# jeremy-collins/sd-video-gen

Hardware: AMD Instinct MI355X
Metric: generated frames/sec at 50 DDIM denoise steps, 512x512 (higher is better)
Workload: dtype fp16; 1 GPU; configs[2]: 1_16_kitti_L1_64 F=64, 64x64 latents -> 512x512 VAE passes, 50-step DDIM; --denoise --denoise_start_step 0, guidance_scale 0; SD-v1.4 UNet at 64x64 latents, VAE enc/dec at 512x512; clips_per_gpu=56, streams_per_gpu=2, pred_frames=1, global_clips=56, parallelism=clip-sharded dp1, weights=seeded random init (SD v1.4 architecture, 1_16_kitti_L1_64)

## Files before the change

### include/svg_hip.h

```cpp
#ifndef SVG_HIP_H
#define SVG_HIP_H

#include <stdint.h>

#ifdef __cplusplus
extern "C" {
#endif

typedef struct svg_ctx svg_ctx;

enum svg_model { SVG_TRANSFORMER = 0, SVG_VAE = 1, SVG_UNET = 2, SVG_CLIP_TEXT = 3, SVG_MINILM = 4, SVG_I3D = 5 };
enum svg_status { SVG_OK = 0, SVG_ERR_RUNTIME = -1, SVG_ERR_INVALID = -2 };

int svg_create(int device_id, svg_ctx** out);
void svg_destroy(svg_ctx* ctx);
const char* svg_last_error(svg_ctx* ctx);
const char* svg_version(void);
void svg_env_refresh(void);

int svg_model_configure(svg_ctx* ctx, int model, const char* kv);
int svg_load_weight(svg_ctx* ctx, int model, const char* name, const float* data,
                    const int64_t* shape, int ndim);
int svg_finalize(svg_ctx* ctx, int model, int64_t* n_params);
const char* svg_model_dtype(svg_ctx* ctx, int model);
// ... 139 lines not shown
  int64_t vt_bs;
  const uint16_t* A2;
  int lda2, k_split;
  float* gn_part;
  float* ln_part;
  int ln_tiles;
} svg_gemm_desc;
int svg_op_gemm_ex(svg_ctx* ctx, const svg_gemm_desc* desc, int* path, void* stream);
int svg_op_gemm_plan(svg_ctx* ctx, const svg_gemm_desc* desc, int* plan);
int svg_op_ff_fused(svg_ctx* ctx, const uint16_t* x, const float* ln_gamma, const float* ln_beta, const float* w1,
                    const float* b1, const float* w2, const float* b2, const uint16_t* residual, uint16_t* out, int M,
                    int C, void* stream);
int svg_op_xattn_fused(svg_ctx* ctx, const uint16_t* x, const uint16_t* a, const uint16_t* r, const float* wp, const float* bp,
                       const float* ln_gamma, const float* ln_beta, const float* wq, const uint16_t* k, const uint16_t* vt, int Lp,
                       const float* wo, const float* bo, uint16_t* out, int M, int rows_per_sample, int L, void* stream);
int svg_op_dropout_mask(svg_ctx* ctx, uint64_t seed, int site, float p, float* out, int64_t n, void* stream);
int svg_op_xf_gemm_tn(svg_ctx* ctx, const float* dY, int ldy, const float* X, int ldx, float* dW, float* db, int M, int N, int K,
                      int accumulate, void* stream);
int svg_op_xf_gemm_nn(svg_ctx* ctx, const float* dY, int ldy, const float* W, float* out, int M, int N, int K, const float* gate,
                      float gate_scale, const float* add, int* splits, void* stream);
int svg_op_xf_relu_drop(svg_ctx* ctx, const float* h, float* r, int64_t n, uint64_t seed, int site, float p, void* stream);
int svg_op_xf_add_ln_train(svg_ctx* ctx, const float* x, const float* r, uint64_t seed, int site, float p, const float* gamma,
                           const float* beta, float* y, float* xhat, float* rstd, int M, int d, float eps, void* stream);
int svg_op_xf_ln_bwd(svg_ctx* ctx, const float* dy, const float* xhat, const float* rstd, const float* gamma, float* dz, float* dz_drop,
                     uint64_t seed, int site, float p, float* dgamma, float* dbeta, int M, int d, int accumulate, void* stream);
int svg_op_xf_attention_train(svg_ctx* ctx, const float* q, int ldq, const float* k, const float* v, int ldk, const float* mask, float* o,
                              float* P, int Tq, int Tk, int B, int heads, int hd, uint64_t seed, int site, float p, void* stream);
int svg_op_xf_attention_bwd(svg_ctx* ctx, const float* dout, const float* q, int ldq, const float* k, const float* v, int ldk,
                            const float* P, float* dq, int lddq, float* dk, float* dv, int lddk, int Tq, int Tk, int B, int heads, int hd,
                            uint64_t seed, int site, float p, void* stream);
// ... 104 lines not shown
int svg_op_conv3x3_gn_f16(svg_ctx* ctx, const uint16_t* x, const float* w_oihw, const float* bias, const float* gamma,
                          const float* beta, uint16_t* conv_out, uint16_t* gn_out, int B, int H, int W, int Cin, int Cout,
                          int groups, float eps, int silu, int* used_epilogue_stats, void* stream);
int svg_op_gemm_lnstats_f16(svg_ctx* ctx, const uint16_t* A, const uint16_t* W, const float* bias, const uint16_t* residual,
                            uint16_t* C, int M, int N, int K, int batch, float* rs, float* rm, int* used, void* stream);
int svg_op_gemm_ex_f16(svg_ctx* ctx, const svg_gemm_desc* desc, int* path, void* stream);
int svg_op_gemm_plan_f16(svg_ctx* ctx, const svg_gemm_desc* desc, int* plan);
int svg_op_gemm_cat_f16(svg_ctx* ctx, const uint16_t* A, const uint16_t* A2, const uint16_t* W, const float* bias, uint16_t* C,
                        int M, int N, int K, int k_split, void* stream);
int svg_op_ff_fused_f16(svg_ctx* ctx, const uint16_t* x, const float* ln_gamma, const float* ln_beta, const float* w1,
                        const float* b1, const float* w2, const float* b2, const uint16_t* residual, uint16_t* out, int M, int C,
                        void* stream);
int svg_op_xattn_fused_f16(svg_ctx* ctx, const uint16_t* x, const uint16_t* a, const uint16_t* r, const float* wp, const float* bp,
                           const float* ln_gamma, const float* ln_beta, const float* wq, const uint16_t* k, const uint16_t* vt, int Lp,
                           const float* wo, const float* bo, uint16_t* out, int M, int rows_per_sample, int L, void* stream);
int svg_op_conv3x3_mx_f16(svg_ctx* ctx, const uint16_t* x, const float* w_oihw, const float* bias, const uint16_t* residual,
                          uint16_t* out, uint8_t* q_out, uint8_t* s_out, int B, int H, int W, int Cin, int Cout, int mode, void* stream);
int svg_op_quant_mx_f16(svg_ctx* ctx, const uint16_t* x, uint8_t* q, uint8_t* scales, int64_t rows, int K, void* stream);
int svg_op_gemm_fp8_f16(svg_ctx* ctx, const uint16_t* A, const uint16_t* W, const float* bias, const uint16_t* residual, void* C,
                        int M, int N, int K, int act, int out_f32, void* stream);
int svg_op_quant_act_mx_f16(svg_ctx* ctx, const uint16_t* x, uint8_t* q, uint8_t* scales, int64_t P, int C, void* stream);
int svg_op_conv3x3_mx_ex_f16(svg_ctx* ctx, const svg_conv_mx_desc* desc, int* path, void* stream);
int svg_op_gemm_fp8_ex_f16(svg_ctx* ctx, const uint16_t* A, const uint16_t* W, const float* bias, const uint16_t* residual, void* C,
                           int M, int N, int K, int act, int out_f32, int ldc, int ldr, int* path, void* stream);
int svg_op_groupnorm_f16(svg_ctx* ctx, const uint16_t* x, const float* gamma, const float* beta, uint16_t* out, int B, int HW,
                         int C, int groups, float eps, int silu, void* stream);
int svg_op_conv3x3_f32s_f16(svg_ctx* ctx, const uint16_t* x, const float* w_oihw, const float* bias, const uint16_t* residual,
                            const float* residual_f32, float* out, const float* gamma, const float* beta, uint16_t* gn_out, int B, int H,
                            int W, int Cin, int Cout, int mode, int groups, float eps, int silu, int* halo_width, int* used_epilogue_stats,
                            void* stream);
// ... 83 lines not shown
```

### sd-video-gen_amd/_lib.py

```python
import ctypes as C
import os

import torch

_HERE = os.path.dirname(os.path.abspath(__file__))
LIB_PATH = os.environ.get("SVG_LIB") or os.path.join(_HERE, "libsvg_hip.so")

SVG_TRANSFORMER, SVG_VAE, SVG_UNET, SVG_CLIP_TEXT, SVG_MINILM, SVG_I3D = 0, 1, 2, 3, 4, 5
SVG_ERR_RUNTIME, SVG_ERR_INVALID = -1, -2
SAMPLERS = {"ddim": 0, "dpmpp_2m": 1, "lms": 2}


def sampler_id(name):
    if name not in SAMPLERS:
        raise ValueError("unknown sampler %r (one of %s)" % (name, ", ".join(SAMPLERS)))
    return SAMPLERS[name]

_lib = None

_vp, _i, _f, _i64 = C.c_void_p, C.c_int, C.c_float, C.c_int64

SVG_TENSOR_PARAM, SVG_TENSOR_GRAD, SVG_TENSOR_EXP_AVG, SVG_TENSOR_EXP_AVG_SQ, SVG_TENSOR_EMA = 0, 1, 2, 3, 4
SVG_BACKWARD_ACCUMULATE = 2

# ... 93 lines not shown
    "svg_sample_loop": [_vp, _i, _vp, _i, _i, _i, _vp, _i, _i, _i, _f, _vp, _vp, _vp],
    "svg_dpmpp_step": [_vp, _vp, _vp, _vp, _vp, _vp, _i64, _i, _i, _i, _vp],
    "svg_lms_coefs": [_i, _i, _vp, _vp, _vp, _vp, _vp],
    "svg_lms_step": [_vp, _vp, _vp, _vp, _vp, _i64, _i, _i, _vp],
    "svg_resize_bilinear_f32": [_vp, _vp, _i, _i, _i, _vp, _i, _i, _vp],
    "svg_resize_nearest_u8": [_vp, _vp, _i, _i, _i, _i, _vp, _i, _i, _vp],
    "svg_op_gemm": [_vp, _vp, _vp, _vp, _vp, _vp, _i, _i, _i, _i, _i, _vp],
    "svg_op_conv3x3": [_vp, _vp, _vp, _vp, _vp, _i, _i, _i, _i, _i, _i, _vp],
    "svg_op_conv3x3_gn": [_vp, _vp, _vp, _vp, _vp, _vp, _vp, _vp, _i, _i, _i, _i, _i, _i, _f, _i, C.POINTER(_i), _vp],
    "svg_op_gemm_lnstats": [_vp, _vp, _vp, _vp, _vp, _vp, _i, _i, _i, _i, _vp, _vp, C.POINTER(_i), _vp],
    "svg_op_gemm_cat": [_vp, _vp, _vp, _vp, _vp, _vp, _i, _i, _i, _i, _vp],
    "svg_op_gemm_ex": [_vp, C.POINTER(GemmDesc), C.POINTER(_i), _vp],
    "svg_op_gemm_plan": [_vp, C.POINTER(GemmDesc), C.POINTER(_i)],
    "svg_op_ff_fused": [_vp, _vp, _vp, _vp, _vp, _vp, _vp, _vp, _vp, _vp, _i, _i, _vp],
    "svg_op_xattn_fused": [_vp, _vp, _vp, _vp, _vp, _vp, _vp, _vp, _vp, _vp, _vp, _i, _vp, _vp, _vp, _i, _i, _i, _vp],
    "svg_op_dropout_mask": [_vp, C.c_uint64, _i, _f, _vp, _i64, _vp],
    "svg_op_xf_gemm_tn": [_vp, _vp, _i, _vp, _i, _vp, _vp, _i, _i, _i, _i, _vp],
    "svg_op_xf_gemm_nn": [_vp, _vp, _i, _vp, _vp, _i, _i, _i, _vp, _f, _vp, C.POINTER(_i), _vp],
    "svg_op_xf_relu_drop": [_vp, _vp, _vp, _i64, C.c_uint64, _i, _f, _vp],
    "svg_op_xf_add_ln_train": [_vp, _vp, _vp, C.c_uint64, _i, _f, _vp, _vp, _vp, _vp, _vp, _i, _i, _f, _vp],
    "svg_op_xf_ln_bwd": [_vp, _vp, _vp, _vp, _vp, _vp, _vp, C.c_uint64, _i, _f, _vp, _vp, _i, _i, _i, _vp],
    "svg_op_xf_attention_train": [_vp, _vp, _i, _vp, _vp, _i, _vp, _vp, _vp, _i, _i, _i, _i, _i, C.c_uint64, _i, _f, _vp],
    "svg_op_xf_attention_bwd": [_vp, _vp, _vp, _i, _vp, _vp, _i, _vp, _vp, _i, _vp, _vp, _i, _i, _i, _i, _i, _i, C.c_uint64, _i, _f, _vp],
    "svg_op_xf_embed_post_train": [_vp, _vp, _vp, _vp, _vp, _i, _vp, _i, _i, _i, _f, C.c_uint64, _i, _f, _vp],
    "svg_op_xf_embed_post_bwd": [_vp, _vp, _vp, _i, _i, _i, _i, _f, C.c_uint64, _i, _f, _vp],
    "svg_op_xf_criterion": [_vp, _vp, _vp, _vp, C.POINTER(_f), _i, _i, _i, _i, _i, _i, _f, _f, _f, _f, _f, _f, _vp],
    "svg_op_conv3d": [_vp, _vp, _i, _i, _i, _i, _i, _vp, _vp, _vp, _i64, _i, _i, _i, C.POINTER(_i), C.POINTER(_i), _i, C.POINTER(_i), _vp],
    "svg_op_pack_conv3d": [_vp, _vp, _vp, _vp, _vp, _vp, _vp, _vp, _vp, _i, _i, _i, _i, _f, _vp],
    "svg_op_maxpool3d_same": [_vp, _vp, _vp, _i64, _i, _i, _i, _i, _i, C.POINTER(_i), C.POINTER(_i), C.POINTER(_i), _vp],
    "svg_op_avgpool_thw": [_vp, _vp, _vp, _i, _i, _i, _i, _i, _vp],
# ... 54 lines not shown
    "svg_op_xf_embed_tokens": [_vp, _vp, _vp, _vp, _vp, _i, _i, _i, _i, _vp],
    "svg_op_xf_embed_bert": [_vp, _vp, _vp, _vp, _vp, _vp, _i, _i, _i, _i, _vp],
    "svg_op_xf_mean_pool_norm": [_vp, _vp, _vp, _vp, _i, _i, _i, _vp],
    "svg_op_xf_walk": [_vp, C.POINTER(WalkStage), _i, _i, _i, C.POINTER(_i), _vp],
    "svg_prof_enable": [_vp, _i],
    "svg_prof_reset": [_vp],
    "svg_prof_report": [_vp, C.c_char_p, _i],
    "svg_workspace_bytes": [_vp],
    "svg_transformer_status": [_vp],
    "svg_workspace_growths": [_vp],
    "svg_reserve_workspace": [_vp, _i64],
    "svg_plan_begin": [_vp],
    "svg_plan_end": [_vp, C.POINTER(_i64)],
    "svg_debug_captures_active": [],
}
for _n in ("gemm", "gemm_ex", "gemm_plan", "conv3x3", "conv3x3_gn", "conv3x3_mx", "conv3x3_mx_ex", "gemm_fp8_ex", "quant_act_mx", "gemm_lnstats", "gemm_cat", "ff_fused", "xattn_fused", "quant_mx", "gemm_fp8", "groupnorm", "layernorm",
           "attention", "attention_ex", "vae_attention", "conv3x3_f32s", "groupnorm_f32", "groupnorm_ex", "groupnorm_mx", "gn_fold_weights", "ln_stats",
           "softmax_rows", "rowsum", "img_to_act", "nchw_to_act", "actf32_pad_h16", "concat_channels", "f32_to_h16", "f32_to_h16_x8", "h16_to_f32",
           "timestep_embed"):
    SIGNATURES["svg_op_%s_f16" % _n] = SIGNATURES["svg_op_" + _n]
SIGNATURES["svg_model_dtype"] = [_vp, _i]
_RESTYPES = {"svg_destroy": None, "svg_env_refresh": None, "svg_model_dtype": C.c_char_p, "svg_last_error": C.c_char_p, "svg_version": C.c_char_p,
             "svg_workspace_bytes": _i64, "svg_workspace_growths": _i64}


def host_cpu_quota():
    n = len(os.sched_getaffinity(0)) if hasattr(os, "sched_getaffinity") else (os.cpu_count() or 1)
    limited = False
    for path in (os.environ.get("SVG_CGROUP_CPU_MAX", "/sys/fs/cgroup/cpu.max"),):
        try:
            q, p = open(path).read().split()
# ... 486 lines not shown
```

### sd-video-gen_amd/csrc/kernels.h

```cpp
#pragma once
#include "common.h"
#include "gemm_tiles.h"

namespace SDNS {

enum AMode { A_DENSE = 0, A_CONV_S1 = 1, A_CONV_S2P1 = 2, A_CONV_S2ASYM = 3, A_CONV_UP2 = 4, A_CONV_SMALLC = 5 };
enum Act { ACT_NONE = 0, ACT_SILU = 1, ACT_GELU = 2, ACT_GEGLU = 3 };

struct GemmArgs {
  const h16* A = nullptr;
  int amode = A_DENSE;
  int lda = 0;
  const h16* A2 = nullptr;
  int lda2 = 0, k_split = 0;
  int H = 0, W = 0, Cin = 0;
  int Ho = 0, Wo = 0;
  const h16* Wt = nullptr;
  int ldb = 0;
  int n_valid = 0;
  void* C = nullptr;
  int ldc = 0;
  int M = 0, N = 0, K = 0;
  int batch = 1;
  int64_t sA = 0, sB = 0, sC = 0;
// ... 59 lines not shown
void pack_conv3x3_mx(const float* w_oihw, uint8_t* q, uint8_t* sc, int O, int I, int Npad, int Cp, hipStream_t s);
struct Fp8ConvPath { int bn = 0, tn_major = 0, workgroups = 0; };
void conv_halo_fp8(svg_ctx* ctx, const uint8_t* A8, const uint8_t* As, const uint8_t* W8, const uint8_t* Ws, int Npad, const GemmArgs& g, hipStream_t s,
                   Fp8ConvPath* path = nullptr);

bool ff_fused_supported(int C, int M);
bool xattn_fused_supported(int C, int heads, int M, int rows_per_sample, int L);
int64_t xattn_kv_pack_elems(int N);
void xattn_pack_q(const float* w, const float* gamma, const float* beta, h16* Wq, float* sq, float* bq, int perm, hipStream_t s);
bool xattn_chain_enabled();
void xattn_pack_o(const float* w, h16* Wo, hipStream_t s);
void xattn_pack_kv(const h16* K, int ldk, int64_t k_bs, const h16* Vt, int ldv, int64_t v_bs, h16* Kp, h16* Vp, int N, int L, hipStream_t s);
void xattn_fused(svg_ctx* ctx, const h16* X, int ldx, const h16* R, int ldr, const h16* Wp, const float* bp, const float* rs, const float* rm,
                 const h16* Wq, const float* sq, const float* bq, const h16* Kp, const h16* Vp, const h16* Wo, const float* bo, h16* out, int ldo,
                 int M, int rows_per_sample, int L, hipStream_t s);
void pack_ff2_perm(const float* w, h16* out, int N, int K, hipStream_t s);
void ff_fused(svg_ctx* ctx, const h16* X, int ldx, const h16* W1, const float* b1, const float* s1,
              const h16* W2p, const float* b2, const h16* residual, int ldr, h16* out, int ldo, int M, hipStream_t s);
void pack_conv3x3(const float* w_oihw, h16* out, int O, int I, int Opad, int Ipad, hipStream_t s);
void pack_linear(const float* w, h16* out, int N, int K, int Npad, hipStream_t s);
void fold_ln_weights(float* w, const float* bias_in, const float* gamma, const float* beta, float* bias_out, int N, int K, hipStream_t s);
void rowsum_h16(const h16* w, float* out, int N, int K, hipStream_t s);
void ln_stats(svg_ctx* ctx, const h16* x, float* rs, float* rm, int M, int C, float eps, hipStream_t s);
void pack_geglu(const float* w, const float* b, h16* wout, float* bout, int F, int K, hipStream_t s);

void ln_finish(svg_ctx* ctx, const float* part, int tiles, float* rs, float* rm, int M, int C, float eps, hipStream_t s);
struct GnStats {
  const float* part = nullptr;
  int tiles_per_sample = 0;
  bool valid() const { return part != nullptr && tiles_per_sample > 0; }
// ... 129 lines not shown
```

### sd-video-gen_amd/csrc/models.h

```cpp
#pragma once
#include "kernels.h"
#include "sampler.h"
#include <algorithm>
#include <initializer_list>
#include <memory>

struct WeightStore {
  std::unordered_map<std::string, Weight> map;
  void put(svg_ctx* ctx, const std::string& name, const float* data, const int64_t* shape, int ndim);
  const Weight& get(const std::string& name) const;
  const Weight& get(const std::string& name, std::initializer_list<int64_t> shape) const;
  bool has(const std::string& name) const { return map.count(name) != 0; }
  void release(const std::string& name);
  void clear();
  int64_t total_params() const;
};

std::unordered_map<std::string, std::vector<int64_t>> parse_kv(const char* kv);

template <typename F>
inline void run_planned(svg_ctx* ctx, F&& body) {
  ctx->arena.reset();
  ctx->arena.dry = true;
  ctx->arena.high = 0;
// ... 175 lines not shown
  void decode(svg_ctx* ctx, const float* z, int N, int h, int w, uint8_t* img_out, int outH, int outW, float* float_out,
              hipStream_t s) override;
};

struct XfBlockW {
  NormW gn, ln1, ln2, ln3;
  PackedLinear proj_in, proj_out, qk1, v1, o1, q2, k2, v2, o2, ff1, ff2;
  PackedLinear qkv1;
  float* proj_in_f32 = nullptr;
  h16* ff2p = nullptr;
  h16* xq = nullptr; float* xq_s = nullptr; float* xq_b = nullptr;
  h16* xqp = nullptr;
  h16* xo = nullptr;
  int C = 0;
};
struct KvCache {
  struct Slot { h16* p = nullptr; int64_t cap = 0; };
  std::vector<Slot> k, vt;
  std::vector<Slot> kp, vp;
  bool valid = false;
};

struct UnetModel : UnetIface {
  KvCache kv;
  std::vector<int> block_out{320, 640, 1280, 1280};
  std::vector<int> attn{1, 1, 1, 0};
  int layers = 2, heads = 8, ctx_dim = 768, groups = 32, in_ch = 4, out_ch = 4;
  int fp8 = 0;
  const char* dtype() const override { return SD_F16 ? "fp16" : "bf16"; }
  int temb_dim = 0;
  PackedLinear time1, time2, temb_all;
  ConvW conv_in, conv_out; NormW norm_out;
  std::vector<std::vector<ResW>> down_res; std::vector<std::vector<XfBlockW>> down_attn; std::vector<ConvW> down_s;
  ResW mid0, mid1; XfBlockW mid_attn;
  std::vector<std::vector<ResW>> up_res; std::vector<std::vector<XfBlockW>> up_attn; std::vector<ConvW> up_s;
  void configure(const char* kv) override;
// ... 60 lines not shown
```

### sd-video-gen_amd/csrc/sd_ops.cpp

```cpp
#include "models.h"
#include "../../include/svg_hip.h"
#include <cstdlib>

#if SD_F16
#define SVG_OP(name) name##_f16
#else
#define SVG_OP(name) name
#endif
#define API_BEGIN try {
#define API_END(ctx)                                   \
  return 0;                                            \
  }                                                    \
  catch (const std::exception& e) { return svg_fail(ctx, e); }

using namespace SDNS;

static ConvW stage_conv(svg_ctx* ctx, const float* w_oihw, const float* bias, int Cin, int Cout, bool mx, hipStream_t s) {
  ConvW cw;
  cw.Cin = Cin; cw.Cout = Cout; cw.Opad = (int)align_up(Cout, 4);
  const int64_t nw = (int64_t)Cout * Cin * 9;
  if (!mx) cw.w = ctx->arena.get<h16>((int64_t)cw.Opad * 9 * Cin);
  float* wdev = ctx->arena.get<float>(nw);
  cw.b = ctx->arena.get<float>(cw.Opad);
  if (mx) {
// ... 311 lines not shown
      xattn_pack_q(wqd, gd, bd, Wq, sq, bq, a ? 1 : 0, s);
      xattn_pack_o(wod, Wo, s);
      xattn_pack_kv((const h16*)k, C, (int64_t)L * C, (const h16*)vt, Lp, (int64_t)C * Lp, kp, vp, N, L, s);
      if (a) {
        HIP_OK(hipMemcpyAsync(wpd, wp, (size_t)C * C * 4, hipMemcpyDefault, s));
        HIP_OK(hipMemcpyAsync(bpd, bp, (size_t)C * 4, hipMemcpyDefault, s));
        pack_linear(wpd, Wp, C, C, C, s);
      }
    }
    if (a) xattn_fused(ctx, (const h16*)a, C, (const h16*)r, C, Wp, bpd, nullptr, nullptr, Wq, sq, bq, kp, vp, Wo, bod, (h16*)out, C, M, rows_per_sample, L, s);
    else xattn_fused(ctx, (const h16*)x, C, nullptr, 0, nullptr, nullptr, nullptr, nullptr, Wq, sq, bq, kp, vp, Wo, bod, (h16*)out, C, M, rows_per_sample, L, s);
  });
  API_END(ctx)
}

int SVG_OP(svg_op_quant_mx)(svg_ctx* ctx, const uint16_t* x, uint8_t* q, uint8_t* scales, int64_t rows, int K, void* stream) {
  API_BEGIN
  quant_mx_h16(ctx, (const h16*)x, K, q, scales, rows, K, (hipStream_t)stream);
  API_END(ctx)
}

int SVG_OP(svg_op_quant_act_mx)(svg_ctx* ctx, const uint16_t* x, uint8_t* q, uint8_t* scales, int64_t P, int C, void* stream) {
  API_BEGIN
  SVG_CHECK(x && q && scales && P > 0 && C > 0 && C % 32 == 0, "quant_act_mx op: P %lld C %d unsupported (C %% 32 must be 0)", (long long)P, C);
  quant_act_mx(ctx, (const h16*)x, C, q, scales, P, (hipStream_t)stream);
  API_END(ctx)
}

int SVG_OP(svg_op_gemm_fp8)(svg_ctx* ctx, const uint16_t* A, const uint16_t* W, const float* bias, const uint16_t* residual, void* C, int M, int N,
                    int K, int act, int out_f32, void* stream) {
// ... 321 lines not shown
```

### sd-video-gen_amd/csrc/sdnet.cpp

```cpp
#include "models.h"
#include <algorithm>
#include <cstdlib>

namespace SDNS {

static int64_t chunk_limit() {
  const int64_t full = (1LL << 31) - 1;
  const int64_t v = svg_env_i64("SVG_CHUNK_LIMIT", full);
  return v > 0 && v < full ? v : full;
}

float* keep_f32(svg_ctx* ctx, WeightStore& ws, const std::string& name, int64_t numel) {
  const Weight& w = ws.get(name);
  SVG_CHECK(w.numel == numel, "weight %s has %lld elements, expected %lld", name.c_str(), (long long)w.numel, (long long)numel);
  return w.f32;
}

ConvW load_conv3x3(svg_ctx* ctx, WeightStore& ws, const std::string& prefix, int Cin, int Cout, hipStream_t s, bool fp8) {
  const Weight& w = ws.get(prefix + ".weight", {Cout, Cin, 3, 3});
  ConvW cw;
  cw.Cout = Cout;
  cw.Opad = (int)align_up(Cout, 4);
  cw.Cin = (Cin < 64) ? 8 : Cin;
  SVG_CHECK(Cin <= 8 || Cin % 64 == 0, "conv %s: Cin=%d must be <= 8 or a multiple of 64", prefix.c_str(), Cin);
// ... 211 lines not shown
void vt_proj_into(svg_ctx* ctx, const PackedLinear& wv, const h16* src, int B, int rows, int rows_pad, int K, h16* vt, hipStream_t s,
                  const float* ln_rs, const float* ln_rm) {
  const int C = wv.N;
  GemmArgs g;
  g.A = wv.w; g.lda = K; g.Wt = src; g.ldb = K; g.M = C; g.N = rows_pad; g.n_valid = rows; g.K = K;
  g.batch = B; g.sA = 0; g.sB = (int64_t)rows * K; g.sC = (int64_t)C * rows_pad;
  g.C = vt; g.ldc = rows_pad;
  SVG_CHECK((wv.ln_s != nullptr) == (ln_rs != nullptr), "vt_proj: LayerNorm-folded weights need the token statistics");
  if (wv.b) { g.bias = wv.b; g.bias_row = 1; }
  if (ln_rs) {
    g.ln_rs = ln_rs; g.ln_rm = ln_rm; g.ln_s = wv.ln_s; g.ln_swapped = 1; g.ln_zstride = rows;
  }
  gemm_auto(ctx, g, s, PK_GEMM);
}

void sd_init_device() {
  gemm_init_device();
  gemm_pp_init_device();
  gemm_ws_init_device();
  vae_attn_init_device();
  conv_halo_init_device();
  ff_fused_init_device();
  xattn_fused_init_device();
  gemm_fp8_init_device();
  conv_halo_fp8_init_device();
}

}
```

### sd-video-gen_amd/csrc/unet.cpp

```cpp
#include "models.h"
#include <algorithm>
#include <chrono>
#include <cstdlib>
#include <thread>

namespace SDNS {

void UnetModel::configure(const char* kv) {
  auto m = parse_kv(kv);
  auto geti = [&](const char* k, int& dst) { if (m.count(k)) dst = (int)m[k][0]; };
  if (m.count("block_out")) { block_out.clear(); for (auto v : m["block_out"]) block_out.push_back((int)v); }
  if (m.count("attn")) { attn.clear(); for (auto v : m["attn"]) attn.push_back((int)v); }
  geti("layers", layers); geti("heads", heads); geti("ctx_dim", ctx_dim); geti("groups", groups);
  geti("in_ch", in_ch); geti("out_ch", out_ch);
  fp8 = 0; geti("fp8", fp8);
  ready = false;
}

namespace {

struct TembCollector {
  std::vector<std::string> prefixes;
  std::vector<int> couts;
  int total = 0;
// ... 346 lines not shown
      if (!fused) {
        linear(ctx, h, C, b.qk1, qk, 2 * C, M, s, stat);
        vt = ctx->arena.get<h16>((int64_t)N * C * HWp);
        vt_proj_into(ctx, b.v1, h, N, HW, HWp, C, vt, s, rs, rm);
      }
      attn_core(qk, 2 * C, qk + C, 2 * C, (int64_t)HW * 2 * C, vt, HWp, (int64_t)C * HWp, ao, C, HW, HW);
      ctx->arena.pop();
    }
    h16* h1 = ctx->arena.get<h16>(P * C);
    const bool xa_one = b.xq && xattn_fused_supported(C, m->heads, M, HW, L);
    const bool xa_chain = xa_one && xattn_chain_enabled() && b.o1.K == C && b.o1.N == C;
    LinearOpts o1, o2;
    o1.residual = h; o1.ldr = C; o1.ln = xa_one ? nullptr : &le;
    if (!xa_chain) linear(ctx, ao, C, b.o1, h1, C, M, s, o1);
    h16* h2 = ctx->arena.get<h16>(P * C);
    if (!xa_one) row_stats(h1);
    {
      ctx->arena.push();
      h16* q = xa_one ? nullptr : ctx->arena.get<h16>(P * C);
      if (!xa_one) linear(ctx, h1, C, b.q2, q, C, M, s, stat);
      const int idx = xf_idx++;
      const int64_t kn = (int64_t)N * L * C, vn = (int64_t)N * C * Lp;
      const bool grow_cache = cache && (SVG_LAUNCHING(ctx) || ctx->plan_only);
      auto kv_buf = [&](std::vector<KvCache::Slot> KvCache::*which, int64_t n) -> h16* {
        if (!cache) return ctx->arena.get<h16>(n);
        std::vector<KvCache::Slot>& v = cache->*which;
        if (grow_cache) {
          if ((int)v.size() <= idx) v.resize(idx + 1);
          if (v[idx].cap < n) { v[idx].p = (h16*)ctx->dalloc(n * sizeof(h16)); v[idx].cap = n; cache->valid = false; }
        }
        if (idx < (int)v.size() && v[idx].p) return v[idx].p;
        return (h16*)(uintptr_t)0x1000;
      };
      h16* k = kv_buf(&KvCache::k, kn);
      h16* vt = kv_buf(&KvCache::vt, vn);
      const int64_t pn = xattn_kv_pack_elems(N);
      h16* kp = xa_one ? kv_buf(&KvCache::kp, pn) : nullptr;
      h16* vp = xa_one ? kv_buf(&KvCache::vp, pn) : nullptr;
      if (!(cache && cache->valid && SVG_LAUNCHING(ctx))) {
        linear(ctx, ctxb, m->ctx_dim, b.k2, k, C, N * L, s);
        vt_proj_into(ctx, b.v2, ctxb, N, L, Lp, m->ctx_dim, vt, s);
        if (xa_one && SVG_LAUNCHING(ctx)) xattn_pack_kv(k, C, (int64_t)L * C, vt, Lp, (int64_t)C * Lp, kp, vp, N, L, s);
      }
      if (xa_chain) xattn_fused(ctx, ao, C, h, C, b.o1.w, b.o1.b, nullptr, nullptr, b.xqp, b.xq_s, b.xq_b, kp, vp, b.xo, b.o2.b, h2, C, M, HW, L, s);
      else if (xa_one) xattn_fused(ctx, h1, C, nullptr, 0, nullptr, nullptr, nullptr, nullptr, b.xq, b.xq_s, b.xq_b, kp, vp, b.xo, b.o2.b, h2, C, M, HW, L, s);
      else attn_core(q, C, k, C, (int64_t)L * C, vt, Lp, (int64_t)C * Lp, ao, C, HW, L);
      ctx->arena.pop();
    }
    o2.residual = h1; o2.ldr = C; o2.ln = &le;
    if (!xa_one) linear(ctx, ao, C, b.o2, h2, C, M, s, o2);
    const bool ff_one = b.ff2p && ff_fused_supported(C, M);
    if (!ff_one) row_stats(h2);
    {
      if (ff_one) {
        ff_fused(ctx, h2, C, b.ff1.w, b.ff1.b, b.ff1.ln_s, b.ff2p, b.ff2.b, h2, C, h, C, M, s);
      } else {
        ctx->arena.push();
        h16* g = ctx->arena.get<h16>((int64_t)M * 4 * C);
        LinearOpts f1, f2;
        f1.act = ACT_GEGLU; f1.ln_rs = rs; f1.ln_rm = rm;
        f2.residual = h2; f2.ldr = C;
        linear(ctx, h2, C, b.ff1, g, 4 * C, M, s, f1);
        linear(ctx, g, 4 * C, b.ff2, h, C, M, s, f2);
        ctx->arena.pop();
      }
// ... 106 lines not shown
}

void UnetModel::sample_loop(svg_ctx* ctx, int sampler, float* z, int N, int h, int w, const float* text_emb, int ctx_len, int num_steps,
                            int start_step, float guidance, const float* noise, float* hist, hipStream_t s) {
  SVG_CHECK(ready, "unet: svg_finalize has not been called");
  const SamplerPlan plan = sampler_plan(sampler, num_steps, start_step);
  SVG_CHECK(start_step == 0 || noise, "ddim: start_step > 0 needs the add_noise draws");
  const int64_t n = (int64_t)N * in_ch * h * w;
  const bool cfg = guidance != 0.f;
  const int NB = cfg ? 2 * N : N;
  const int64_t sites = cfg ? svg_env_i64("SVG_FP8_SITES_GUIDED", kFp8SitesGuided) : -1;

  const int graph_env = (int)svg_env_i64("SVG_DDIM_GRAPH", 1);
  const bool use_graph = graph_env && s != nullptr && !ctx->prof && !hist && (num_steps - start_step) >= 3;

  auto body = [&]() {
    kv.valid = false;
    const bool own_input = cfg || plan.scaled_input;
    float* tvec = ctx->arena.get<float>(NB);
    float* zin = own_input ? ctx->arena.get<float>((cfg ? 2 : 1) * n) : nullptr;
    float* eps = ctx->arena.get<float>((int64_t)NB * n / N);
    float* tab = ctx->arena.get<float>((int64_t)plan.table.size());
    int* idx = ctx->arena.get<int>(1);
    float* state = plan.state_buffers ? ctx->arena.get<float>(plan.state_buffers * n) : nullptr;
    if (SVG_LAUNCHING(ctx)) {
      if (plan.add_noise) add_noise(z, noise, z, n, plan.noise_sa, plan.noise_s1a, s);
      if (plan.scaled_input) lms_input(z, z, nullptr, n, sampler_scale(plan.z_scale), s);
      if (hist) HIP_OK(hipMemcpyAsync(hist, z, n * sizeof(float), hipMemcpyDeviceToDevice, s));
      if (use_graph) {
        HIP_OK(hipMemcpyAsync(tab, plan.table.data(), plan.table.size() * sizeof(float), hipMemcpyHostToDevice, s));
        const int first = start_step;
        HIP_OK(hipMemcpyAsync(idx, &first, sizeof(int), hipMemcpyHostToDevice, s));
        HIP_OK(hipStreamSynchronize(s));
      }
    }
    auto one_step = [&](int i, bool tabled) {
      const SamplerRowArg row = tabled ? sampler_row_at(tab, idx) : sampler_row(plan.row(i));
      ctx->arena.push();
      if (SVG_LAUNCHING(ctx)) {
        if (tabled) sampler_tvec(tvec, NB, tab, idx, s);
        else fill_f32(tvec, NB, plan.timestep(i), s);
        if (plan.scaled_input) {
          lms_input(z, zin, cfg ? zin + n : nullptr, n, row, s);
        } else if (cfg) {
          HIP_OK(hipMemcpyAsync(zin, z, n * sizeof(float), hipMemcpyDeviceToDevice, s));
          HIP_OK(hipMemcpyAsync(zin + n, z, n * sizeof(float), hipMemcpyDeviceToDevice, s));
        }
      }
      std::unique_ptr<ProfScope> step_scope;
// ... 44 lines not shown
```

Baseline: 18.28 frames/s.

## Fold shared-context cross-attention Q/K and V/O products into precomputed weights

Adds a folded cross-attention path for when every sample in the batch shares the same text context, which is checked on the GPU once per sampling call. It precomputes per-head Wq·Kᵀ score weights and Wo·V output weights once per cache build. Each denoise step then replaces the Q projection, the attention and the O projection with one GEMM, a small softmax over 80 slots and a second GEMM, and the K/V projection runs for one sample instead of N. By default this applies only to 1280-channel levels; it adds a device-to-host flag readback at the start of sampling and fp16 rounding of the folded weights.

```diff
diff --git a/include/svg_hip.h b/include/svg_hip.h
--- a/include/svg_hip.h
+++ b/include/svg_hip.h
@@ -177,6 +177,9 @@
 int svg_op_xattn_fused(svg_ctx* ctx, const uint16_t* x, const uint16_t* a, const uint16_t* r, const float* wp, const float* bp,
                        const float* ln_gamma, const float* ln_beta, const float* wq, const uint16_t* k, const uint16_t* vt, int Lp,
                        const float* wo, const float* bo, uint16_t* out, int M, int rows_per_sample, int L, void* stream);
+int svg_op_xattn_folded(svg_ctx* ctx, const uint16_t* x, const float* ln_gamma, const float* ln_beta, const float* wq, const uint16_t* k,
+                        const uint16_t* vt, int Lp, const float* wo, const float* bo, uint16_t* out, int M, int rows_per_sample, int C,
+                        int heads, int L, int folded, void* stream);
 int svg_op_dropout_mask(svg_ctx* ctx, uint64_t seed, int site, float p, float* out, int64_t n, void* stream);
 int svg_op_xf_gemm_tn(svg_ctx* ctx, const float* dY, int ldy, const float* X, int ldx, float* dW, float* db, int M, int N, int K,
                       int accumulate, void* stream);
@@ -311,6 +314,9 @@
 int svg_op_xattn_fused_f16(svg_ctx* ctx, const uint16_t* x, const uint16_t* a, const uint16_t* r, const float* wp, const float* bp,
                            const float* ln_gamma, const float* ln_beta, const float* wq, const uint16_t* k, const uint16_t* vt, int Lp,
                            const float* wo, const float* bo, uint16_t* out, int M, int rows_per_sample, int L, void* stream);
+int svg_op_xattn_folded_f16(svg_ctx* ctx, const uint16_t* x, const float* ln_gamma, const float* ln_beta, const float* wq, const uint16_t* k,
+                            const uint16_t* vt, int Lp, const float* wo, const float* bo, uint16_t* out, int M, int rows_per_sample, int C,
+                            int heads, int L, int folded, void* stream);
 int svg_op_conv3x3_mx_f16(svg_ctx* ctx, const uint16_t* x, const float* w_oihw, const float* bias, const uint16_t* residual,
                           uint16_t* out, uint8_t* q_out, uint8_t* s_out, int B, int H, int W, int Cin, int Cout, int mode, void* stream);
 int svg_op_quant_mx_f16(svg_ctx* ctx, const uint16_t* x, uint8_t* q, uint8_t* scales, int64_t rows, int K, void* stream);
diff --git a/sd-video-gen_amd/_lib.py b/sd-video-gen_amd/_lib.py
--- a/sd-video-gen_amd/_lib.py
+++ b/sd-video-gen_amd/_lib.py
@@ -131,6 +131,7 @@
     "svg_op_gemm_plan": [_vp, C.POINTER(GemmDesc), C.POINTER(_i)],
     "svg_op_ff_fused": [_vp, _vp, _vp, _vp, _vp, _vp, _vp, _vp, _vp, _vp, _i, _i, _vp],
     "svg_op_xattn_fused": [_vp, _vp, _vp, _vp, _vp, _vp, _vp, _vp, _vp, _vp, _vp, _i, _vp, _vp, _vp, _i, _i, _i, _vp],
+    "svg_op_xattn_folded": [_vp, _vp, _vp, _vp, _vp, _vp, _vp, _i, _vp, _vp, _vp, _i, _i, _i, _i, _i, _i, _vp],
     "svg_op_dropout_mask": [_vp, C.c_uint64, _i, _f, _vp, _i64, _vp],
     "svg_op_xf_gemm_tn": [_vp, _vp, _i, _vp, _i, _vp, _vp, _i, _i, _i, _i, _vp],
     "svg_op_xf_gemm_nn": [_vp, _vp, _i, _vp, _vp, _i, _i, _i, _vp, _f, _vp, C.POINTER(_i), _vp],
@@ -215,7 +216,7 @@
     "svg_plan_end": [_vp, C.POINTER(_i64)],
     "svg_debug_captures_active": [],
 }
-for _n in ("gemm", "gemm_ex", "gemm_plan", "conv3x3", "conv3x3_gn", "conv3x3_mx", "conv3x3_mx_ex", "gemm_fp8_ex", "quant_act_mx", "gemm_lnstats", "gemm_cat", "ff_fused", "xattn_fused", "quant_mx", "gemm_fp8", "groupnorm", "layernorm",
+for _n in ("gemm", "gemm_ex", "gemm_plan", "conv3x3", "conv3x3_gn", "conv3x3_mx", "conv3x3_mx_ex", "gemm_fp8_ex", "quant_act_mx", "gemm_lnstats", "gemm_cat", "ff_fused", "xattn_fused", "xattn_folded", "quant_mx", "gemm_fp8", "groupnorm", "layernorm",
            "attention", "attention_ex", "vae_attention", "conv3x3_f32s", "groupnorm_f32", "groupnorm_ex", "groupnorm_mx", "gn_fold_weights", "ln_stats",
            "softmax_rows", "rowsum", "img_to_act", "nchw_to_act", "actf32_pad_h16", "concat_channels", "f32_to_h16", "f32_to_h16_x8", "h16_to_f32",
            "timestep_embed"):
diff --git a/sd-video-gen_amd/csrc/kernels.h b/sd-video-gen_amd/csrc/kernels.h
--- a/sd-video-gen_amd/csrc/kernels.h
+++ b/sd-video-gen_amd/csrc/kernels.h
@@ -97,6 +97,12 @@
 void xattn_fused(svg_ctx* ctx, const h16* X, int ldx, const h16* R, int ldr, const h16* Wp, const float* bp, const float* rs, const float* rm,
                  const h16* Wq, const float* sq, const float* bq, const h16* Kp, const h16* Vp, const h16* Wo, const float* bo, h16* out, int ldo,
                  int M, int rows_per_sample, int L, hipStream_t s);
+constexpr int XF_SLOTS = 80;
+bool xattn_folded_supported(int C, int heads, int L);
+void ctx_differs(const float* emb, int B, int64_t per_sample, int* flag, hipStream_t s);
+void xattn_fold_s(const h16* wq, const float* bq, const h16* k, int ldk, h16* ws, float* bs, float* ss, int C, int heads, int L, hipStream_t s);
+void xattn_fold_vo(const h16* wo, const h16* vt, int ldv, h16* wvo, int C, int heads, int L, hipStream_t s);
+void xattn_softmax(svg_ctx* ctx, const float* scores, h16* p, int M, int heads, int L, hipStream_t s);
 void pack_ff2_perm(const float* w, h16* out, int N, int K, hipStream_t s);
 void ff_fused(svg_ctx* ctx, const h16* X, int ldx, const h16* W1, const float* b1, const float* s1,
               const h16* W2p, const float* b2, const h16* residual, int ldr, h16* out, int ldo, int M, hipStream_t s);
diff --git a/sd-video-gen_amd/csrc/models.h b/sd-video-gen_amd/csrc/models.h
--- a/sd-video-gen_amd/csrc/models.h
+++ b/sd-video-gen_amd/csrc/models.h
@@ -213,12 +213,25 @@
   h16* xo = nullptr;
   int C = 0;
 };
+struct XattnFolded { PackedLinear s, vo; };
 struct KvCache {
   struct Slot { h16* p = nullptr; int64_t cap = 0; };
   std::vector<Slot> k, vt;
   std::vector<Slot> kp, vp;
   bool valid = false;
-};
+  bool shared = false;
+  int* differs = nullptr;
+  std::vector<XattnFolded> fold;
+};
+constexpr int kXattnFoldDefault = 2;
+int xattn_fold_levels();
+static inline bool xattn_fold_level_on(int C) { return (xattn_fold_levels() >> (C >= 1280 ? 1 : 0)) & 1; }
+XattnFolded xattn_folded_bind(int C, int heads, h16* ws, float* bs, float* ss, h16* wvo, float* bo);
+void xattn_folded_build(svg_ctx* ctx, const PackedLinear& q2, const PackedLinear& o2, const h16* k, const h16* vt, int Lp, int heads, int L,
+                        const XattnFolded& f, hipStream_t s);
+struct LnEmit;
+void xattn_folded(svg_ctx* ctx, const h16* x, const XattnFolded& f, const float* rs, const float* rm, const h16* residual, h16* out, int M,
+                  int heads, int L, LnEmit* ln, hipStream_t s);
 
 struct UnetModel : UnetIface {
   KvCache kv;
diff --git a/sd-video-gen_amd/csrc/sd_ops.cpp b/sd-video-gen_amd/csrc/sd_ops.cpp
--- a/sd-video-gen_amd/csrc/sd_ops.cpp
+++ b/sd-video-gen_amd/csrc/sd_ops.cpp
@@ -349,6 +349,64 @@
   API_END(ctx)
 }
 
+int SVG_OP(svg_op_xattn_folded)(svg_ctx* ctx, const uint16_t* x, const float* ln_gamma, const float* ln_beta, const float* wq, const uint16_t* k,
+                                const uint16_t* vt, int Lp, const float* wo, const float* bo, uint16_t* out, int M, int rows_per_sample, int C,
+                                int heads, int L, int folded, void* stream) {
+  API_BEGIN
+  hipStream_t s = (hipStream_t)stream;
+  SVG_CHECK(xattn_folded_supported(C, heads, L) && rows_per_sample >= 1 && M >= 1 && M % rows_per_sample == 0 && Lp >= L && Lp % 8 == 0,
+            "xattn_folded op: C %d, %d heads, L %d (Lp %d), M %d in samples of %d rows is not supported", C, heads, L, Lp, M, rows_per_sample);
+  const int N = M / rows_per_sample;
+  run_planned(ctx, [&]() {
+    float* wqd = ctx->arena.get<float>((int64_t)C * C);
+    float* wod = ctx->arena.get<float>((int64_t)C * C);
+    float* gd = ctx->arena.get<float>(C);
+    float* bd = ctx->arena.get<float>(C);
+    PackedLinear q2, o2;
+    q2.N = o2.N = q2.K = o2.K = q2.n_valid = o2.n_valid = C;
+    q2.w = ctx->arena.get<h16>((int64_t)C * C); q2.b = ctx->arena.get<float>(C); q2.ln_s = ctx->arena.get<float>(C);
+    o2.w = ctx->arena.get<h16>((int64_t)C * C); o2.b = ctx->arena.get<float>(C);
+    float* rs = ctx->arena.get<float>(M + 8);
+    float* rm = ctx->arena.get<float>(M + 8);
+    if (SVG_LAUNCHING(ctx)) {
+      HIP_OK(hipMemcpyAsync(wqd, wq, (size_t)C * C * 4, hipMemcpyDefault, s));
+      HIP_OK(hipMemcpyAsync(wod, wo, (size_t)C * C * 4, hipMemcpyDefault, s));
+      HIP_OK(hipMemcpyAsync(gd, ln_gamma, (size_t)C * 4, hipMemcpyDefault, s));
+      HIP_OK(hipMemcpyAsync(bd, ln_beta, (size_t)C * 4, hipMemcpyDefault, s));
+      HIP_OK(hipMemcpyAsync(o2.b, bo, (size_t)C * 4, hipMemcpyDefault, s));
+      HIP_OK(hipMemsetAsync(q2.b, 0, (size_t)C * 4, s));
+      fold_ln_weights(wqd, q2.b, gd, bd, q2.b, C, C, s);
+      pack_linear(wqd, q2.w, C, C, C, s);
+      rowsum_h16(q2.w, q2.ln_s, C, C, s);
+      pack_linear(wod, o2.w, C, C, C, s);
+    }
+    ln_stats(ctx, (const h16*)x, rs, rm, M, C, 1e-5f, s);
+    if (folded) {
+      const int64_t NS = (int64_t)heads * XF_SLOTS;
+      const XattnFolded f = xattn_folded_bind(C, heads, ctx->arena.get<h16>(NS * C), ctx->arena.get<float>(NS), ctx->arena.get<float>(NS),
+                                              ctx->arena.get<h16>(NS * C), o2.b);
+      xattn_folded_build(ctx, q2, o2, (const h16*)k, (const h16*)vt, Lp, heads, L, f, s);
+      xattn_folded(ctx, (const h16*)x, f, rs, rm, (const h16*)x, (h16*)out, M, heads, L, nullptr, s);
+    } else {
+      h16* q = ctx->arena.get<h16>((int64_t)M * C);
+      h16* ao = ctx->arena.get<h16>((int64_t)M * C);
+      LinearOpts lq, lo;
+      lq.ln_rs = rs; lq.ln_rm = rm;
+      linear(ctx, (const h16*)x, C, q2, q, C, M, s, lq);
+      AttnArgs a;
+      a.q = q; a.k = (const h16*)k; a.vt = (const h16*)vt; a.out = ao;
+      a.B = N; a.heads = heads; a.Sq = rows_per_sample; a.Skv = L; a.d = C / heads;
+      a.ldq = C; a.ldk = C; a.ldvt = Lp; a.ldo = C;
+      a.qb = (int64_t)rows_per_sample * C; a.kb = (int64_t)L * C; a.vtb = (int64_t)C * Lp; a.ob = (int64_t)rows_per_sample * C;
+      a.scale = 1.f / sqrtf((float)a.d);
+      attention(ctx, a, s);
+      lo.residual = (const h16*)x; lo.ldr = C;
+      linear(ctx, ao, C, o2, (h16*)out, C, M, s, lo);
+    }
+  });
+  API_END(ctx)
+}
+
 int SVG_OP(svg_op_quant_mx)(svg_ctx* ctx, const uint16_t* x, uint8_t* q, uint8_t* scales, int64_t rows, int K, void* stream) {
   API_BEGIN
   quant_mx_h16(ctx, (const h16*)x, K, q, scales, rows, K, (hipStream_t)stream);
diff --git a/sd-video-gen_amd/csrc/sdnet.cpp b/sd-video-gen_amd/csrc/sdnet.cpp
--- a/sd-video-gen_amd/csrc/sdnet.cpp
+++ b/sd-video-gen_amd/csrc/sdnet.cpp
@@ -249,6 +249,42 @@
   gemm_auto(ctx, g, s, PK_GEMM);
 }
 
+int xattn_fold_levels() { return (int)svg_env_i64("SVG_XATTN_FOLD", kXattnFoldDefault); }
+
+XattnFolded xattn_folded_bind(int C, int heads, h16* ws, float* bs, float* ss, h16* wvo, float* bo) {
+  XattnFolded f;
+  const int NS = heads * XF_SLOTS;
+  f.s.w = ws; f.s.b = bs; f.s.ln_s = ss; f.s.N = NS; f.s.K = C; f.s.n_valid = NS;
+  f.vo.w = wvo; f.vo.b = bo; f.vo.N = C; f.vo.K = NS; f.vo.n_valid = C;
+  return f;
+}
+
+void xattn_folded_build(svg_ctx* ctx, const PackedLinear& q2, const PackedLinear& o2, const h16* k, const h16* vt, int Lp, int heads, int L,
+                        const XattnFolded& f, hipStream_t s) {
+  const int C = q2.K;
+  SVG_CHECK(xattn_folded_supported(C, heads, L) && q2.N == C && o2.N == C && o2.K == C && q2.ln_s && f.s.K == C && f.s.N == heads * XF_SLOTS && Lp >= L,
+            "xattn_folded: C %d, %d heads, L %d (row stride %d) cannot be folded", C, heads, L, Lp);
+  if (!SVG_LAUNCHING(ctx)) return;
+  ProfScope ps(ctx, PK_GEMM, s, 4.0 * f.s.N * C * (C / heads), 0, "xattn_fold");
+  xattn_fold_s(q2.w, q2.b, k, C, f.s.w, f.s.b, f.s.ln_s, C, heads, L, s);
+  xattn_fold_vo(o2.w, vt, Lp, f.vo.w, C, heads, L, s);
+}
+
+void xattn_folded(svg_ctx* ctx, const h16* x, const XattnFolded& f, const float* rs, const float* rm, const h16* residual, h16* out, int M,
+                  int heads, int L, LnEmit* ln, hipStream_t s) {
+  const int C = f.s.K, NS = f.s.N;
+  ctx->arena.push();
+  float* sc = ctx->arena.get<float>((int64_t)M * NS);
+  h16* p = ctx->arena.get<h16>((int64_t)M * NS);
+  LinearOpts a, b;
+  a.out_f32 = 1; a.ln_rs = rs; a.ln_rm = rm;
+  linear(ctx, x, C, f.s, sc, NS, M, s, a);
+  xattn_softmax(ctx, sc, p, M, heads, L, s);
+  b.residual = residual; b.ldr = C; b.ln = ln;
+  linear(ctx, p, NS, f.vo, out, C, M, s, b);
+  ctx->arena.pop();
+}
+
 void sd_init_device() {
   gemm_init_device();
   gemm_pp_init_device();
diff --git a/sd-video-gen_amd/csrc/unet.cpp b/sd-video-gen_amd/csrc/unet.cpp
--- a/sd-video-gen_amd/csrc/unet.cpp
+++ b/sd-video-gen_amd/csrc/unet.cpp
@@ -384,11 +384,19 @@
     o1.residual = h; o1.ldr = C; o1.ln = xa_one ? nullptr : &le;
     if (!xa_chain) linear(ctx, ao, C, b.o1, h1, C, M, s, o1);
     h16* h2 = ctx->arena.get<h16>(P * C);
+    const bool fold_ok = !xa_one && cache && xattn_fold_level_on(C) && xattn_folded_supported(C, m->heads, L);
+    const bool xa_fold = fold_ok && cache->shared;
+    if (fold_ok && !xa_fold && ctx->arena.dry) {
+      ctx->arena.push();
+      ctx->arena.get<float>(P * m->heads * XF_SLOTS);
+      ctx->arena.get<h16>(P * m->heads * XF_SLOTS);
+      ctx->arena.pop();
+    }
     if (!xa_one) row_stats(h1);
     {
       ctx->arena.push();
-      h16* q = xa_one ? nullptr : ctx->arena.get<h16>(P * C);
-      if (!xa_one) linear(ctx, h1, C, b.q2, q, C, M, s, stat);
+      h16* q = xa_one || xa_fold ? nullptr : ctx->arena.get<h16>(P * C);
+      if (!xa_one && !xa_fold) linear(ctx, h1, C, b.q2, q, C, M, s, stat);
       const int idx = xf_idx++;
       const int64_t kn = (int64_t)N * L * C, vn = (int64_t)N * C * Lp;
       const bool grow_cache = cache && (SVG_LAUNCHING(ctx) || ctx->plan_only);
@@ -407,18 +415,30 @@
       const int64_t pn = xattn_kv_pack_elems(N);
       h16* kp = xa_one ? kv_buf(&KvCache::kp, pn) : nullptr;
       h16* vp = xa_one ? kv_buf(&KvCache::vp, pn) : nullptr;
+      if (fold_ok && grow_cache && (xa_fold || ctx->plan_only)) {
+        if ((int)cache->fold.size() <= idx) cache->fold.resize(idx + 1);
+        if (!cache->fold[idx].s.w) {
+          const int64_t NS = m->heads * XF_SLOTS;
+          cache->fold[idx] = xattn_folded_bind(C, m->heads, (h16*)ctx->dalloc(NS * C * sizeof(h16)), (float*)ctx->dalloc(NS * sizeof(float)),
+                                               (float*)ctx->dalloc(NS * sizeof(float)), (h16*)ctx->dalloc(NS * C * sizeof(h16)), b.o2.b);
+          cache->valid = false;
+        }
+      }
       if (!(cache && cache->valid && SVG_LAUNCHING(ctx))) {
-        linear(ctx, ctxb, m->ctx_dim, b.k2, k, C, N * L, s);
-        vt_proj_into(ctx, b.v2, ctxb, N, L, Lp, m->ctx_dim, vt, s);
+        const int Nk = xa_fold ? 1 : N;
+        linear(ctx, ctxb, m->ctx_dim, b.k2, k, C, Nk * L, s);
+        vt_proj_into(ctx, b.v2, ctxb, Nk, L, Lp, m->ctx_dim, vt, s);
         if (xa_one && SVG_LAUNCHING(ctx)) xattn_pack_kv(k, C, (int64_t)L * C, vt, Lp, (int64_t)C * Lp, kp, vp, N, L, s);
+        if (xa_fold && SVG_LAUNCHING(ctx)) xattn_folded_build(ctx, b.q2, b.o2, k, vt, Lp, m->heads, L, cache->fold[idx], s);
       }
       if (xa_chain) xattn_fused(ctx, ao, C, h, C, b.o1.w, b.o1.b, nullptr, nullptr, b.xqp, b.xq_s, b.xq_b, kp, vp, b.xo, b.o2.b, h2, C, M, HW, L, s);
       else if (xa_one) xattn_fused(ctx, h1, C, nullptr, 0, nullptr, nullptr, nullptr, nullptr, b.xq, b.xq_s, b.xq_b, kp, vp, b.xo, b.o2.b, h2, C, M, HW, L, s);
+      else if (xa_fold) xattn_folded(ctx, h1, cache->fold[idx], rs, rm, h1, h2, M, m->heads, L, &le, s);
       else attn_core(q, C, k, C, (int64_t)L * C, vt, Lp, (int64_t)C * Lp, ao, C, HW, L);
       ctx->arena.pop();
     }
     o2.residual = h1; o2.ldr = C; o2.ln = &le;
-    if (!xa_one) linear(ctx, ao, C, b.o2, h2, C, M, s, o2);
+    if (!xa_one && !xa_fold) linear(ctx, ao, C, b.o2, h2, C, M, s, o2);
     const bool ff_one = b.ff2p && ff_fused_supported(C, M);
     if (!ff_one) row_stats(h2);
     {
@@ -555,8 +575,16 @@
   const int graph_env = (int)svg_env_i64("SVG_DDIM_GRAPH", 1);
   const bool use_graph = graph_env && s != nullptr && !ctx->prof && !hist && (num_steps - start_step) >= 3;
 
+  auto fold_candidate = [&](int L) {
+    auto ok = [&](const XfBlockW& b) { return xattn_fold_level_on(b.C) && xattn_folded_supported(b.C, heads, L); };
+    bool any = ok(mid_attn);
+    for (auto& v : down_attn) for (auto& b : v) any |= ok(b);
+    for (auto& v : up_attn) for (auto& b : v) any |= ok(b);
+    return any;
+  };
   auto body = [&]() {
     kv.valid = false;
+    kv.shared = false;
     const bool own_input = cfg || plan.scaled_input;
     float* tvec = ctx->arena.get<float>(NB);
     float* zin = own_input ? ctx->arena.get<float>((cfg ? 2 : 1) * n) : nullptr;
@@ -568,12 +596,21 @@
       if (plan.add_noise) add_noise(z, noise, z, n, plan.noise_sa, plan.noise_s1a, s);
       if (plan.scaled_input) lms_input(z, z, nullptr, n, sampler_scale(plan.z_scale), s);
       if (hist) HIP_OK(hipMemcpyAsync(hist, z, n * sizeof(float), hipMemcpyDeviceToDevice, s));
+      int differs = 0;
+      const bool detect = fold_candidate(ctx_len);
+      if (detect && NB > 1) {
+        if (!kv.differs) kv.differs = (int*)ctx->dalloc(sizeof(int));
+        ctx_differs(text_emb, NB, (int64_t)ctx_len * ctx_dim, kv.differs, s);
+        HIP_OK(hipMemcpyAsync(&differs, kv.differs, sizeof(int), hipMemcpyDeviceToHost, s));
+        if (!use_graph) HIP_OK(hipStreamSynchronize(s));
+      }
       if (use_graph) {
         HIP_OK(hipMemcpyAsync(tab, plan.table.data(), plan.table.size() * sizeof(float), hipMemcpyHostToDevice, s));
         const int first = start_step;
         HIP_OK(hipMemcpyAsync(idx, &first, sizeof(int), hipMemcpyHostToDevice, s));
         HIP_OK(hipStreamSynchronize(s));
       }
+      kv.shared = detect && differs == 0;
     }
     auto one_step = [&](int i, bool tabled) {
       const SamplerRowArg row = tabled ? sampler_row_at(tab, idx) : sampler_row(plan.row(i));
diff --git a/sd-video-gen_amd/csrc/xattn_folded.hip b/sd-video-gen_amd/csrc/xattn_folded.hip
--- /dev/null
+++ b/sd-video-gen_amd/csrc/xattn_folded.hip
@@ -0,0 +1,122 @@
+#include "kernels.h"
+
+namespace SDNS {
+
+namespace {
+
+__global__ void __launch_bounds__(256) ctx_differs_kernel(const uint32_t* __restrict__ e, int64_t per_sample, int64_t total, int* __restrict__ flag) {
+  bool diff = false;
+  for (int64_t i = (int64_t)blockIdx.x * blockDim.x + threadIdx.x; i < total; i += (int64_t)gridDim.x * blockDim.x)
+    diff |= e[per_sample + i] != e[i % per_sample];
+  if (diff) flag[0] = 1;
+}
+
+constexpr int FJ = 8;
+__global__ void __launch_bounds__(256) xattn_fold_s_kernel(const h16* __restrict__ wq, const float* __restrict__ bq, const h16* __restrict__ k, int ldk,
+                                                           h16* __restrict__ ws, float* __restrict__ bs, int C, int d0, int L, float scale) {
+  const int n0 = blockIdx.x * FJ, h = n0 / XF_SLOTS, j0 = n0 - h * XF_SLOTS;
+  const int c = blockIdx.y * 256 + threadIdx.x;
+  const h16* wr = wq + (int64_t)h * d0 * C;
+  if (c < C) {
+    float acc[FJ];
+#pragma unroll
+    for (int t = 0; t < FJ; ++t) acc[t] = 0.f;
+    for (int d = 0; d < d0; ++d) {
+      const float w = (float)wr[(int64_t)d * C + c];
+#pragma unroll
+      for (int t = 0; t < FJ; ++t)
+        if (j0 + t < L) acc[t] = fmaf(w, (float)k[(int64_t)(j0 + t) * ldk + h * d0 + d], acc[t]);
+    }
+#pragma unroll
+    for (int t = 0; t < FJ; ++t) ws[(int64_t)(n0 + t) * C + c] = (h16)(acc[t] * scale);
+  }
+  if (blockIdx.y == 0 && threadIdx.x < FJ) {
+    const int j = j0 + threadIdx.x;
+    float acc = 0.f;
+    if (j < L)
+      for (int d = 0; d < d0; ++d) acc = fmaf(bq[h * d0 + d], (float)k[(int64_t)j * ldk + h * d0 + d], acc);
+    bs[n0 + threadIdx.x] = acc * scale;
+  }
+}
+
+__global__ void __launch_bounds__(256) xattn_fold_vo_kernel(const h16* __restrict__ wo, const h16* __restrict__ vt, int ldv, h16* __restrict__ wvo, int C,
+                                                            int d0, int NS, int L) {
+  const int c = blockIdx.x;
+  for (int n = threadIdx.x; n < NS; n += blockDim.x) {
+    const int h = n / XF_SLOTS, j = n - h * XF_SLOTS;
+    float acc = 0.f;
+    if (j < L) {
+      const h16* wr = wo + (int64_t)c * C + h * d0;
+      const h16* vr = vt + (int64_t)h * d0 * ldv + j;
+      for (int d = 0; d < d0; ++d) acc = fmaf((float)wr[d], (float)vr[(int64_t)d * ldv], acc);
+    }
+    wvo[(int64_t)c * NS + n] = (h16)acc;
+  }
+}
+
+__global__ void __launch_bounds__(256) xattn_softmax_kernel(const float* __restrict__ sc, h16* __restrict__ p, int64_t waves, int L) {
+  const int64_t w = (int64_t)blockIdx.x * 4 + (threadIdx.x >> 6);
+  const int lane = threadIdx.x & 63;
+  if (w >= waves) return;
+  const bool act = lane < XF_SLOTS / 2;
+  const int j = 2 * lane;
+  float v0 = -INFINITY, v1 = -INFINITY;
+  if (act) {
+    const float2 v = *(const float2*)(sc + w * XF_SLOTS + j);
+    if (j < L) v0 = v.x;
+    if (j + 1 < L) v1 = v.y;
+  }
+  float m = fmaxf(v0, v1);
+  for (int o = 32; o > 0; o >>= 1) m = fmaxf(m, __shfl_xor(m, o));
+  constexpr float kLog2e = 1.4426950408889634f;
+  const float e0 = __builtin_amdgcn_exp2f((v0 - m) * kLog2e), e1 = __builtin_amdgcn_exp2f((v1 - m) * kLog2e);
+  float l = e0 + e1;
+  for (int o = 32; o > 0; o >>= 1) l += __shfl_xor(l, o);
+  const float inv = 1.f / l;
+  if (act) {
+    typedef h16 h16x2 __attribute__((ext_vector_type(2)));
+    h16x2 r;
+    r.x = (h16)(e0 * inv); r.y = (h16)(e1 * inv);
+    *(h16x2*)(p + w * XF_SLOTS + j) = r;
+  }
+}
+
+}
+
+bool xattn_folded_supported(int C, int heads, int L) {
+  return C >= 640 && heads >= 1 && C % heads == 0 && heads * XF_SLOTS <= C && L >= 1 && L <= XF_SLOTS;
+}
+
+void ctx_differs(const float* emb, int B, int64_t per_sample, int* flag, hipStream_t s) {
+  HIP_OK(hipMemsetAsync(flag, 0, sizeof(int), s));
+  if (B < 2) return;
+  const int64_t total = (int64_t)(B - 1) * per_sample;
+  hipLaunchKernelGGL(ctx_differs_kernel, dim3((unsigned)std::min<int64_t>(cdiv(total, 256), 1024)), dim3(256), 0, s, (const uint32_t*)emb, per_sample,
+                     total, flag);
+  check_launch("ctx_differs");
+}
+
+void xattn_fold_s(const h16* wq, const float* bq, const h16* k, int ldk, h16* ws, float* bs, float* ss, int C, int heads, int L, hipStream_t s) {
+  const int d0 = C / heads, NS = heads * XF_SLOTS;
+  hipLaunchKernelGGL(xattn_fold_s_kernel, dim3(NS / FJ, cdiv(C, 256)), dim3(256), 0, s, wq, bq, k, ldk, ws, bs, C, d0, L, 1.f / sqrtf((float)d0));
+  check_launch("xattn_fold_s");
+  rowsum_h16(ws, ss, NS, C, s);
+}
+
+void xattn_fold_vo(const h16* wo, const h16* vt, int ldv, h16* wvo, int C, int heads, int L, hipStream_t s) {
+  hipLaunchKernelGGL(xattn_fold_vo_kernel, dim3(C), dim3(256), 0, s, wo, vt, ldv, wvo, C, C / heads, heads * XF_SLOTS, L);
+  check_launch("xattn_fold_vo");
+}
+
+void xattn_softmax(svg_ctx* ctx, const float* scores, h16* p, int M, int heads, int L, hipStream_t s) {
+  SVG_CHECK(L >= 1 && L <= XF_SLOTS && M >= 1 && heads >= 1, "xattn_softmax: M %d heads %d L %d unsupported", M, heads, L);
+  if (!SVG_LAUNCHING(ctx)) return;
+  const int64_t waves = (int64_t)M * heads;
+  char tag[64];
+  snprintf(tag, sizeof(tag), "xattn_folded_M%d_H%d_L%d", M, heads, L);
+  ProfScope ps(ctx, PK_ATTN, s, 0, (double)waves * XF_SLOTS * 6.0, tag);
+  hipLaunchKernelGGL(xattn_softmax_kernel, dim3((unsigned)cdiv(waves, 4)), dim3(256), 0, s, scores, p, waves, L);
+  check_launch("xattn_softmax");
+}
+
+}
```

Result: no change. 18.38 frames/s, median of 6 (+0.5%).
